# MrTornado24/FENeRF

Hardware: NVIDIA H100
Metric: rendered faces/sec at 128px x 24 samples/ray (higher is better)
Workload: dtype f16 operands / f32 accumulate (wgmma) + f32 refinement

## Files before the change

### fenerf_b200/csrc/siren_fast.cu

```cuda
#include "siren_fast.cuh"

namespace fn {

int siren_fast_label_launch(const void* args, int blocks, cudaStream_t st);
int siren_fast_hd_launch(const void* args, int blocks, bool label_film, cudaStream_t st);
int siren_fast_grid_launch(const void* args, int blocks, cudaStream_t st);
int siren_fast_bridge_launch(const void* args, int blocks, cudaStream_t st);
int siren_fast_debug_launch(const void* args, int blocks, bool label_film, bool feature_head, int variant, cudaStream_t st);

namespace {

std::atomic<int> g_variant{0};
unsigned long long* g_trace = nullptr;
int g_trace_ctas = 0;

bool build_loads(const FnLayout& L, FastArgs& A, bool sigma_only) {
    A.n_loads = 0;
    auto push = [&](size_t src, uint32_t bytes) {
        if (A.n_loads < MAX_LOADS) A.loads[A.n_loads] = Load{(uint32_t)src, bytes};
        ++A.n_loads;
    };
    push(L.first_img, 2 * CHUNK);
    if (L.grid_trunk) push(L.first_img_lo, 2 * CHUNK);
    for (int l = 0; l < L.n_hidden; ++l) {
        if (l == L.trunk_hidden) {
            push(L.head_img, 4 * HEAD_CHUNK);
            if (sigma_only) return A.n_loads <= MAX_LOADS;
        }
        if (L.bridge && l == L.color0) {
            push(L.color0_ximg, 2 * CHUNK);
            continue;
        }
        push(L.hid_img[l], 2 * CHUNK);
        push(L.hid_img[l] + 2 * CHUNK, 2 * CHUNK);
        if (l == L.label_layer) push(L.label.img, (uint32_t)FN_HEAD_IMG_BYTES(L.label.img_rows));
        if (l == L.color0) push(L.color0_ximg, 2 * CHUNK);
        push(L.hid_img[l] + 4 * CHUNK, 2 * CHUNK);
        push(L.hid_img[l] + 6 * CHUNK, 2 * CHUNK);
    }
    push(L.rgb.img, (uint32_t)FN_HEAD_IMG_BYTES(L.rgb.img_rows));
    return A.n_loads <= MAX_LOADS;
}

}

int siren_fast_debug_variant(int variant, unsigned long long* trace, int trace_ctas) {
    FN_REQUIRE(variant >= 0 && variant <= 3, "unknown point-network variant %d", variant);
    FN_REQUIRE(variant < 2 || (trace && trace_ctas >= 1), "a timeline variant needs its trace buffer");
    g_trace = trace;
    g_trace_ctas = trace_ctas;
    g_variant.store(variant);
    return 0;
}

int siren_points_fast(const FnLayout& L, const unsigned char* packed, const float* points, const float* dirs, const float* film,
                      int batch, long long ppb, int dir_group, int lock_dirs, float* out, int sigma_only, cudaStream_t st,
                      float* sigma_out) {
    static_assert(sizeof(FastArgs) <= 4000, "kernel parameter block too large");
    static_assert(SMEM_TOTAL <= 232448, "one CTA per SM: 227 KB of shared memory");
    static_assert(FN_HEAD_IMG_BYTES(FN_FEAT) == SLOT_BYTES, "a feature-head image is one ring slot");
    const bool trunk_only = L.feature_head && sigma_only;
    const bool feature_head = L.feature_head && !trunk_only, label_film = L.label_film && !trunk_only;
    FN_REQUIRE(L.trunk_hidden >= 1 && L.n_hidden - L.color0 >= 1, "field needs >= 2 trunk and >= 1 colour layers");
    FN_REQUIRE(L.sigma_row < 32, "the fast path packs labels and sigma into one 32-column head (label_dim <= 31)");
    FN_REQUIRE(L.rgb.img < 0xFFFFFFFFull && L.label.img < 0xFFFFFFFFull && L.first_img_lo < 0xFFFFFFFFull,
               "packed weight images beyond 4 GB");
    FN_REQUIRE(((uintptr_t)film & 15) == 0, "the FiLM table must be 16-byte aligned");
    if (L.wo_dir && !sigma_only)
        return fail(FENERF_E_UNSUPPORTED, "FENERF_FIELD_WO_DIR: the wgmma colour branch is not accurate for this field (its "
                    "first colour layer amplifies the fp16 trunk's error to ~2e-2 in rgb); render it with "
                    "FENERF_PRECISION_EXACT or FENERF_PRECISION_SPLIT (the density alone runs in any precision)");
    FastArgs a;
    memset(&a, 0, sizeof(a));
    FN_REQUIRE(build_loads(L, a, sigma_only != 0), "field too deep for the weight stream");
    a.sigma_only = sigma_only ? 1 : 0;
    a.L = L; a.packed = packed; a.points = points; a.dirs = dirs; a.film = film; a.out = out; a.sigma_out = sigma_out;
    a.ppb = ppb; a.tiles_per_batch = (ppb + TILE - 1) / TILE; a.n_tiles = a.tiles_per_batch * batch;
    a.dir_group = dir_group < 1 ? 1 : dir_group; a.lock_dirs = lock_dirs;
    if (a.n_tiles <= 0) return 0;
    FN_REQUIRE(ppb % a.dir_group == 0, "points_per_batch %lld not a multiple of dir_group %d", ppb, a.dir_group);
    const long long n_pairs = (a.n_tiles + 1) / 2;
    static std::atomic<int> attr_set[kMaxDevices];
    const int blocks = (int)(n_pairs < (long long)num_sms() ? n_pairs : (long long)num_sms());
    if (const int variant = g_variant.load()) {
        FN_REQUIRE(!L.grid_trunk && !L.bridge,
                   "the debug point-network variants do not cover fields with the grid in the trunk or a bridge");
        a.trace = g_trace;
        a.trace_ctas = g_trace_ctas;
        return siren_fast_debug_launch(&a, blocks, label_film, feature_head, variant, st);
    }
    if (L.grid_trunk) return siren_fast_grid_launch(&a, blocks, st);
    if (L.bridge) return siren_fast_bridge_launch(&a, blocks, st);
    if (feature_head) return siren_fast_hd_launch(&a, blocks, label_film, st);
    if (label_film) return siren_fast_label_launch(&a, blocks, st);
    FN_CUDA_OK(ensure_dynamic_smem(siren_fast_kernel<false>, attr_set, (int)SMEM_TOTAL));
    siren_fast_kernel<false><<<blocks, NTHREADS, SMEM_TOTAL, st>>>(a);
    FN_LAUNCH_OK("siren_fast_kernel");
    return 0;
}

}
```

### fenerf_b200/csrc/siren_fast.cuh

```cuda
#pragma once
#include "common.cuh"
#include "siren_common.cuh"
#include "sm90.cuh"

namespace fn {

namespace {

using namespace sm90;

constexpr int TILE = 64;
constexpr int NTHREADS = 384;
constexpr int PROD_WARP = 8;
constexpr int RING = 6;
constexpr uint32_t SLOT_BYTES = 32768;
constexpr int XSTRIDE = 72;
constexpr uint32_t SMEM_X = RING * SLOT_BYTES;
constexpr int FRING = 2;
constexpr uint32_t FILM_BYTES = 2 * FN_H * 4;
constexpr uint32_t SMEM_FILM = SMEM_X + 2 * TILE * XSTRIDE * 2;
constexpr uint32_t SMEM_BAR = SMEM_FILM + 2 * FRING * FILM_BYTES;
constexpr uint32_t SMEM_TOTAL = SMEM_BAR + 16 * RING + 16 + 16 * 2 * FRING;
constexpr uint32_t SMEM_XLO = SMEM_TOTAL;
constexpr int XLO_STRIDE = 32;
constexpr uint32_t SMEM_TOTAL_GRID = SMEM_XLO + 2 * TILE * XLO_STRIDE * 2;
constexpr int RING_SPLIT = 4;
constexpr uint32_t ALO_CHUNK = TILE * FN_KCHUNK * 2;
constexpr uint32_t ALO_BYTES = (FN_H / FN_KCHUNK) * ALO_CHUNK;
constexpr uint32_t SPLIT_SMEM_ALO = RING_SPLIT * SLOT_BYTES;
constexpr uint32_t SPLIT_SMEM_X = SPLIT_SMEM_ALO + 2 * ALO_BYTES;
constexpr uint32_t SPLIT_SMEM_FILM = SPLIT_SMEM_X + 2 * TILE * XSTRIDE * 2;
constexpr uint32_t SPLIT_SMEM_BAR = SPLIT_SMEM_FILM + 2 * FRING * FILM_BYTES;
constexpr uint32_t SPLIT_SMEM_XLO = SPLIT_SMEM_BAR + 16 * RING_SPLIT + 16 + 16 * 2 * FRING;
constexpr uint32_t SMEM_TOTAL_SPLIT = SPLIT_SMEM_XLO + 2 * TILE * XLO_STRIDE * 2;
constexpr int MAX_LOADS = 72;
constexpr int MAX_LOADS_SPLIT = 132;
constexpr uint32_t CHUNK = 16384;
constexpr uint32_t HEAD_CHUNK = 32 * 128;
constexpr uint32_t RGB_CHUNK = 8 * 128;
constexpr uint32_t FEAT_CHUNK = FN_FEAT * 128;
#ifndef FENERF_SOFT_SIN_EVERY
#define FENERF_SOFT_SIN_EVERY 0
#endif
constexpr int kSoftSinEvery = FENERF_SOFT_SIN_EVERY;
constexpr int kSoftSinSplit = 4;
constexpr int TRACE_CAP = 1024;
constexpr int TRACE_WARPS = 11;
enum TraceEvent {
    TR_PAIR = 1, TR_TURN_WAIT, TR_TURN_DONE, TR_ACQ_WAIT, TR_ACQ_DONE, TR_COMMIT, TR_MMA_DONE, TR_EPI_DONE,
    TR_FILM_WAIT, TR_FILM_DONE, TR_EMPTY_WAIT, TR_EMPTY_DONE,
};
enum TraceGroup { TG_FIRST = 0, TG_HIDDEN, TG_COLOR0, TG_TRUNK_HEAD, TG_LABEL_LAYER, TG_LABEL_HEAD, TG_OUT_HEAD };

__device__ __forceinline__ float soft_sinf(float a) {
    const float k = fmaf(a, 0.159154943f, 12582912.f);
    const float n = k - 12582912.f;
    float r = fmaf(-n, 6.28318548f, a);
    r = fmaf(-n, -1.74845553e-7f, r);
    const float r2 = r * r;
    float p = -2.041572245e-08f;
    p = fmaf(p, r2, 2.701100129e-06f);
    p = fmaf(p, r2, -1.980991656e-04f);
    p = fmaf(p, r2, 8.332454599e-03f);
    p = fmaf(p, r2, -1.666656137e-01f);
    p = fmaf(p, r2, 9.999996424e-01f);
    return r * p;
}

struct Load {
    uint32_t src;
    uint32_t bytes;
};

template <int kMaxLoads>
struct FastArgsT {
    Load loads[kMaxLoads];
    int n_loads;
    FnLayout L;
    const unsigned char* packed;
    const float* points;
    const float* dirs;
    const float* film;
    float* out;
    float* sigma_out;
    long long ppb, tiles_per_batch, n_tiles;
    int dir_group, lock_dirs;
    int sigma_only;
    unsigned long long* trace;
    int trace_ctas;
};
using FastArgs = FastArgsT<MAX_LOADS>;
using SplitArgs = FastArgsT<MAX_LOADS_SPLIT>;

__device__ __forceinline__ void wg_bar(int wg) { asm volatile("bar.sync %0, 128;" ::"r"(1 + wg) : "memory"); }

template <bool kLabelFilm, bool kFeatureHead = false, int kSoftSin = kSoftSinEvery, bool kTrace = false,
          bool kGridTrunk = false, bool kBridge = false, bool kSplit = false>
__global__ void __launch_bounds__(NTHREADS, 1)
    siren_fast_kernel(const __grid_constant__ FastArgsT<kSplit ? MAX_LOADS_SPLIT : MAX_LOADS> a) {
    constexpr int RING = kSplit ? RING_SPLIT : fn::RING;
    constexpr uint32_t SMEM_X = kSplit ? SPLIT_SMEM_X : fn::SMEM_X;
    constexpr uint32_t SMEM_FILM = kSplit ? SPLIT_SMEM_FILM : fn::SMEM_FILM;
    constexpr uint32_t SMEM_BAR = kSplit ? SPLIT_SMEM_BAR : fn::SMEM_BAR;
    constexpr uint32_t SMEM_XLO = kSplit ? SPLIT_SMEM_XLO : fn::SMEM_XLO;
    extern __shared__ __align__(1024) unsigned char smem[];
    const uint32_t sbase = smem_u32(smem);
    const int warp = threadIdx.x >> 5, lane = threadIdx.x & 31;
    const uint32_t bar_full = sbase + SMEM_BAR, bar_empty = bar_full + 8 * RING, bar_turn = bar_empty + 8 * RING;
    const uint32_t bar_ffull = bar_turn + 16, bar_fempty = bar_ffull + 8 * 2 * FRING;
    unsigned long long* tbuf = nullptr;
    uint32_t tn = 0;
    if constexpr (kTrace)
        if (lane == 0 && (int)blockIdx.x < a.trace_ctas) tbuf = a.trace + ((size_t)blockIdx.x * TRACE_WARPS + warp) * TRACE_CAP;
    auto trace = [&](int kind, int group = 0) {
        if constexpr (kTrace)
            if (tbuf && tn < TRACE_CAP)
                tbuf[tn++] = ((unsigned long long)kind << 56) | ((unsigned long long)group << 48) |
                             ((unsigned long long)clock64() & ((1ull << 48) - 1));
    };
    if (threadIdx.x == 0) {
        for (int i = 0; i < RING; ++i) {
            mbar_init(bar_full + 8 * i, 1);
            mbar_init(bar_empty + 8 * i, 8);
        }
        for (int g = 0; g < 2; ++g) mbar_init(bar_turn + 8 * g, 4);
        for (int e = 0; e < 2 * FRING; ++e) {
            mbar_init(bar_ffull + 8 * e, 32);
            mbar_init(bar_fempty + 8 * e, 4);
        }
        fence_barrier_init();
    }
    __syncthreads();
    const long long n_pairs = (a.n_tiles + 1) / 2;

    if (warp >= PROD_WARP) {
        asm volatile("setmaxnreg.dec.sync.aligned.u32 40;\n" ::: "memory");
        if (warp == PROD_WARP && lane == 0) {
            uint32_t it = 0;
            for (long long pair = blockIdx.x; pair < n_pairs; pair += gridDim.x)
                for (int i = 0; i < a.n_loads; ++i, ++it) {
                    const uint32_t slot = it % RING;
                    trace(TR_EMPTY_WAIT);
                    mbar_wait(bar_empty + 8 * slot, ((it / RING) & 1u) ^ 1u);
                    trace(TR_EMPTY_DONE);
                    mbar_arrive_expect_tx(bar_full + 8 * slot, a.loads[i].bytes);
                    bulk_g2s(sbase + slot * SLOT_BYTES, a.packed + a.loads[i].src, a.loads[i].bytes, bar_full + 8 * slot);
                }
        } else if (warp == PROD_WARP + 1 || warp == PROD_WARP + 2) {
            const int g = warp - PROD_WARP - 1;
            const int n_film = 1 + (a.sigma_only ? a.L.trunk_hidden : a.L.n_hidden);
            uint32_t it = 0;
            for (long long pair = blockIdx.x; pair < n_pairs; pair += gridDim.x) {
                const long long tile = pair * 2 + g;
                const long long b = tile < a.n_tiles ? tile / a.tiles_per_batch : 0;
                const float* film_b = a.film + (size_t)b * a.L.n_film * 2 * FN_H;
                for (int i = 0; i < n_film; ++i, ++it) {
                    const uint32_t e = g * FRING + it % FRING;
                    const float2* row = reinterpret_cast<const float2*>(film_b + (size_t)i * 2 * FN_H);
                    const float2* bias = reinterpret_cast<const float2*>(a.packed + (i == 0 ? a.L.first_b : a.L.hid_b[i - 1]));
                    float4* dst = reinterpret_cast<float4*>(smem + SMEM_FILM + e * FILM_BYTES);
                    trace(TR_EMPTY_WAIT);
                    mbar_wait(bar_fempty + 8 * e, ((it / FRING) & 1u) ^ 1u);
                    trace(TR_EMPTY_DONE);
#pragma unroll 1
                    for (int k = 0; k < FN_H / 64; ++k) {
                        const int cp = lane + 32 * k;
                        const float2 f = __ldg(row + cp), p = __ldg(row + FN_H / 2 + cp), bb = __ldg(bias + cp);
                        if constexpr (kSplit) {
                            const float us = __ldg(reinterpret_cast<const float*>(a.packed + a.L.split_scale) +
                                                   FN_SPLIT_SCALES + i);
                            dst[cp] = make_float4(f.x * us, f.y * us, fmaf(f.x, bb.x, p.x), fmaf(f.y, bb.y, p.y));
                        } else {
                            dst[cp] = make_float4(f.x, f.y, fmaf(f.x, bb.x, p.x), fmaf(f.y, bb.y, p.y));
                        }
                    }
                    mbar_arrive(bar_ffull + 8 * e);
                }
            }
        }
        return;
    }

    asm volatile("setmaxnreg.inc.sync.aligned.u32 232;\n" ::: "memory");
    const int wg = warp >> 2, q = lane & 3;
    const int tid = threadIdx.x & 127;
    const int r0 = (warp & 3) * 16 + (lane >> 2);
    const FnLayout& L = a.L;
    const int C = L.out_dim;
    const float* sigma_w = reinterpret_cast<const float*>(a.packed + L.sigma_w);
    const float* label_w = reinterpret_cast<const float*>(a.packed + L.label_w);
    const int trunk_labels = (kLabelFilm || kFeatureHead) ? 0 : L.trunk_labels;
    const int sigma_row = kFeatureHead ? FN_FEAT_SIGMA_ROW : L.sigma_row;
    const int rgb_rows = kFeatureHead ? FN_FEAT : L.rgb.w_rows;
    const int label_rows = kFeatureHead ? FN_FEAT : L.label.w_rows;
    __half* xs = reinterpret_cast<__half*>(smem + SMEM_X) + wg * TILE * XSTRIDE;
    uint32_t it = 0;
    auto acquire = [&](uint32_t& slot) -> uint32_t {
        slot = it % RING;
        trace(TR_ACQ_WAIT);
        mbar_wait(bar_full + 8 * slot, (it / RING) & 1u);
        trace(TR_ACQ_DONE);
        ++it;
        return sbase + slot * SLOT_BYTES;
    };
    auto release = [&](uint32_t slot) {
        __syncwarp();
        if (lane == 0) mbar_arrive(bar_empty + 8 * slot);
    };
    uint32_t turns = 0;
    uint32_t fit = 0;
    auto film_acquire = [&]() -> const float4* {
        const uint32_t e = wg * FRING + fit % FRING;
        trace(TR_FILM_WAIT);
        mbar_wait(bar_ffull + 8 * e, (fit / FRING) & 1u);
        trace(TR_FILM_DONE);
        return reinterpret_cast<const float4*>(smem + SMEM_FILM + e * FILM_BYTES);
    };
    auto film_release = [&]() {
        const uint32_t e = wg * FRING + fit % FRING;
        ++fit;
        __syncwarp();
        if (lane == 0) mbar_arrive(bar_fempty + 8 * e);
    };
    auto turn_begin = [&]() {
        trace(TR_TURN_WAIT);
        mbar_wait(bar_turn + 8 * wg, (turns & 1u) ^ (wg == 0 ? 1u : 0u));
        trace(TR_TURN_DONE);
    };
    auto turn_end = [&](int group) {
        trace(TR_COMMIT, group);
        ++turns;
        __syncwarp();
        if (lane == 0) mbar_arrive(bar_turn + 8 * (wg ^ 1));
    };
    auto xfrag = [&](int s, uint32_t (&f)[4]) {
        const __half* p = xs + r0 * XSTRIDE + 16 * s + 2 * q;
        f[0] = *reinterpret_cast<const uint32_t*>(p);
        f[1] = *reinterpret_cast<const uint32_t*>(p + 8 * XSTRIDE);
        f[2] = *reinterpret_cast<const uint32_t*>(p + 8);
        f[3] = *reinterpret_cast<const uint32_t*>(p + 8 * XSTRIDE + 8);
    };

    for (long long pair = blockIdx.x; pair < n_pairs; pair += gridDim.x) {
        const long long tile = pair * 2 + wg;
        const bool tile_ok = tile < a.n_tiles;
        const long long b = tile_ok ? tile / a.tiles_per_batch : 0;
        const long long p0 = tile_ok ? (tile % a.tiles_per_batch) * TILE : a.ppb;
        trace(TR_PAIR);

        wg_bar(wg);
        if (tid < TILE) {
            float pos[3] = {0.f, 0.f, 0.f}, dir[3] = {0.f, 0.f, 0.f};
            const long long pp = p0 + tid;
            const bool valid = pp < a.ppb;
            if (valid) {
                const long long ff = b * a.ppb + pp;
#pragma unroll
                for (int i = 0; i < 3; ++i) pos[i] = __fmul_rn(a.points[ff * 3 + i], L.input_scale);
                if (a.lock_dirs) dir[2] = -1.f;
                else {
                    const long long di = b * (a.ppb / a.dir_group) + pp / a.dir_group;
#pragma unroll
                    for (int i = 0; i < 3; ++i) dir[i] = a.dirs[di * 3 + i];
                }
            }
            __align__(16) __half slots[64];
#pragma unroll
            for (int i = 0; i < 64; ++i) slots[i] = __float2half_rn(0.f);
#pragma unroll
            for (int i = 0; i < 3; ++i) {
                __half hi, lo;
                split_f16(pos[i], hi, lo);
                slots[FN_SLOT_POS + i] = hi; slots[FN_SLOT_POS + 3 + i] = lo; slots[FN_SLOT_POS + 6 + i] = hi;
                split_f16(dir[i], hi, lo);
                slots[FN_SLOT_DIR + i] = hi; slots[FN_SLOT_DIR + 3 + i] = lo; slots[FN_SLOT_DIR + 6 + i] = hi;
            }
            if constexpr (kGridTrunk || kSplit) {
                __align__(16) __half lo[32];
#pragma unroll
                for (int i = 0; i < 32; ++i) lo[i] = __float2half_rn(0.f);
                if (valid && (kGridTrunk || (L.grid_channels > 0 && !a.sigma_only))) {
                    float feat[32];
                    grid_features32(reinterpret_cast<const float*>(a.packed + L.grid), L.grid_res, pos[0], pos[1], pos[2], feat);
#pragma unroll
                    for (int i = 0; i < 32; ++i) split_f16(feat[i], slots[FN_SLOT_FEAT + i], lo[i]);
                }
                __half* xlo = reinterpret_cast<__half*>(smem + SMEM_XLO) + (wg * TILE + tid) * XLO_STRIDE;
#pragma unroll
                for (int i = 0; i < 4; ++i) reinterpret_cast<uint4*>(xlo)[i] = reinterpret_cast<const uint4*>(lo)[i];
            } else if (L.grid_channels > 0 && valid && !a.sigma_only) {
                float feat[32];
                grid_features32_h(reinterpret_cast<const __half*>(a.packed + L.grid16), L.grid_res, pos[0], pos[1], pos[2], feat);
#pragma unroll
                for (int i = 0; i < 32; ++i) slots[FN_SLOT_FEAT + i] = __float2half_rn(feat[i]);
            }
#pragma unroll
            for (int i = 0; i < 8; ++i)
                reinterpret_cast<uint4*>(xs + tid * XSTRIDE)[i] = reinterpret_cast<const uint4*>(slots)[i];
        }
        wg_bar(wg);

        uint32_t act[16][4];
        uint32_t nxt[8][4];
        float d[64];
        auto film_epi = [&](const float4* fs, int h, uint32_t (&dst)[8][4]) {
#pragma unroll
            for (int j = 0; j < 16; ++j) {
                const float4 e = fs[64 * h + 4 * j + q];
                const bool soft = kSoftSin > 0 && j % (kSoftSin > 0 ? kSoftSin : 1) == kSoftSin - 1;
                auto sn = [soft](float x) { return soft ? soft_sinf(x) : __sinf(x); };
                dst[j >> 1][(j & 1) * 2] = pack_half2(sn(fmaf(e.x, d[4 * j], e.z)), sn(fmaf(e.y, d[4 * j + 1], e.w)));
                dst[j >> 1][(j & 1) * 2 + 1] = pack_half2(sn(fmaf(e.x, d[4 * j + 2], e.z)), sn(fmaf(e.y, d[4 * j + 3], e.w)));
            }
            trace(TR_EPI_DONE);
        };
        auto act_hi = [&]() -> uint32_t (&)[8][4] { return *reinterpret_cast<uint32_t (*)[8][4]>(&act[8]); };
        auto film_epi_split = [&](const float4* fs, int h, uint32_t (&dst)[8][4], uint32_t (&lo)[8][4]) {
#pragma unroll
            for (int j = 0; j < 16; ++j) {
                const float4 e = fs[64 * h + 4 * j + q];
#pragma unroll
                for (int rr = 0; rr < 2; ++rr) {
                    const float s0 = soft_sinf(fmaf(e.x, d[4 * j + 2 * rr], e.z));
                    const float s1 = soft_sinf(fmaf(e.y, d[4 * j + 2 * rr + 1], e.w));
                    const __half2 hi = __floats2half2_rn(s0, s1);
                    const float2 hf = __half22float2(hi);
                    dst[j >> 1][(j & 1) * 2 + rr] = *reinterpret_cast<const uint32_t*>(&hi);
                    lo[j >> 1][(j & 1) * 2 + rr] = pack_half2(s0 - hf.x, s1 - hf.y);
                }
            }
            trace(TR_EPI_DONE);
        };
        const uint32_t alo_base = sbase + SPLIT_SMEM_ALO + wg * ALO_BYTES;
        auto alo_desc = [&](int s) { return desc_kmajor(alo_base + (s >> 2) * ALO_CHUNK + 32 * (s & 3)); };
        auto alo_store = [&](const uint32_t (&lo0)[8][4], const uint32_t (&lo1)[8][4]) {
            wg_bar(wg);
            unsigned char* base = smem + SPLIT_SMEM_ALO + wg * ALO_BYTES;
#pragma unroll
            for (int h = 0; h < 2; ++h)
#pragma unroll
                for (int j = 0; j < 16; ++j) {
                    const int col = 128 * h + 8 * j + 2 * q;
#pragma unroll
                    for (int rr = 0; rr < 2; ++rr)
                        *reinterpret_cast<uint32_t*>(base + (col >> 6) * ALO_CHUNK + fn_sw128_offset(r0 + 8 * rr, col & 63)) =
                            (h ? lo1 : lo0)[j >> 1][(j & 1) * 2 + rr];
                }
            fence_async_smem();
            wg_bar(wg);
        };
        uint32_t lo0[8][4], lo1[8][4];

        {
            uint32_t xf[4], slot, slot_lo = 0, w_lo = 0;
            uint32_t xg[2][4], xl[2][4];
            const float4* fs = nullptr;
            xfrag(0, xf);
            if constexpr (kGridTrunk) {
                const __half* xlo = reinterpret_cast<const __half*>(smem + SMEM_XLO) + wg * TILE * XLO_STRIDE;
#pragma unroll
                for (int s = 0; s < 2; ++s) {
                    xfrag(2 + s, xg[s]);
                    const __half* p = xlo + r0 * XLO_STRIDE + 16 * s + 2 * q;
                    xl[s][0] = *reinterpret_cast<const uint32_t*>(p);
                    xl[s][1] = *reinterpret_cast<const uint32_t*>(p + 8 * XLO_STRIDE);
                    xl[s][2] = *reinterpret_cast<const uint32_t*>(p + 8);
                    xl[s][3] = *reinterpret_cast<const uint32_t*>(p + 8 * XLO_STRIDE + 8);
                }
            }
            const uint32_t w = acquire(slot);
            if constexpr (kGridTrunk) w_lo = acquire(slot_lo);
#pragma unroll
            for (int h = 0; h < 2; ++h) {
                turn_begin();
                wg_fence();
                mma_rs_n128(d, xf, desc_kmajor(w + h * CHUNK), 0u);
                if constexpr (kGridTrunk)
#pragma unroll
                    for (int s = 0; s < 2; ++s) {
                        mma_rs_n128(d, xg[s], desc_kmajor(w + h * CHUNK + 32 * (2 + s)), 1u);
                        mma_rs_n128(d, xl[s], desc_kmajor(w + h * CHUNK + 32 * (2 + s)), 1u);
                        mma_rs_n128(d, xg[s], desc_kmajor(w_lo + h * CHUNK + 32 * (2 + s)), 1u);
                    }
                wg_commit();
                turn_end(TG_FIRST);
                wg_wait<0>();
                trace(TR_MMA_DONE);
                fence_regs(d);
                fence_regs(xf);
                if constexpr (kGridTrunk) { fence_regs(xg); fence_regs(xl); }
                if (h == 0) fs = film_acquire();
                if constexpr (kSplit) {
                    if (h == 0) film_epi_split(fs, 0, nxt, lo0);
                    else film_epi_split(fs, 1, act_hi(), lo1);
                } else {
                    if (h == 0) film_epi(fs, 0, nxt);
                    else film_epi(fs, 1, act_hi());
                }
            }
            release(slot);
            if constexpr (kGridTrunk) release(slot_lo);
            film_release();
            if constexpr (kSplit) alo_store(lo0, lo1);
#pragma unroll
            for (int s = 0; s < 8; ++s)
#pragma unroll
                for (int i = 0; i < 4; ++i) act[s][i] = nxt[s][i];
        }

        bool stop = false;
        for (int l = 0; l < L.n_hidden && !stop; ++l) {
            if (l == L.trunk_hidden) {
                float dh[16];
                uint32_t slot, slot_lo = 0, w_lo = 0;
                const uint32_t w = acquire(slot);
                if constexpr (kSplit) w_lo = acquire(slot_lo);
                turn_begin();
                wg_fence();
#pragma unroll
                for (int c = 0; c < 4; ++c)
#pragma unroll
                    for (int k = 0; k < 4; ++k) mma_rs_n32(dh, act[4 * c + k], desc_kmajor(w + c * HEAD_CHUNK + 32 * k), (c | k) ? 1u : 0u);
                if constexpr (kSplit)
#pragma unroll
                    for (int c = 0; c < 4; ++c)
#pragma unroll
                        for (int k = 0; k < 4; ++k) {
                            mma_ss_n32(dh, alo_desc(4 * c + k), desc_kmajor(w + c * HEAD_CHUNK + 32 * k), 1u);
                            mma_rs_n32(dh, act[4 * c + k], desc_kmajor(w_lo + c * HEAD_CHUNK + 32 * k), 1u);
                        }
                wg_commit();
                turn_end(TG_TRUNK_HEAD);
                wg_wait<0>();
                trace(TR_MMA_DONE);
                fence_regs(dh);
                fence_regs(act);
                release(slot);
                if constexpr (kSplit) {
                    release(slot_lo);
                    const float us = __ldg(reinterpret_cast<const float*>(a.packed + L.split_scale) + FN_SPLIT_SCALES +
                                           L.n_hidden + 1);
#pragma unroll
                    for (int i = 0; i < 16; ++i) dh[i] *= us;
                }
                const float* lb = label_w + FENERF_MAX_LABEL * FN_H;
#pragma unroll
                for (int rr = 0; rr < 2; ++rr) {
                    const long long pnt = p0 + r0 + 8 * rr;
                    if (pnt >= a.ppb) continue;
                    const long long flat = b * a.ppb + pnt;
#pragma unroll
                    for (int i = 0; i < 4; ++i)
#pragma unroll
                        for (int e = 0; e < 2; ++e) {
                            const int o = 8 * i + 2 * q + e;
                            const float v = dh[4 * i + 2 * rr + e];
                            if (o < trunk_labels) {
                                if (!a.sigma_only) a.out[flat * C + o] = fmaf(v, __ldg(lb + FENERF_MAX_LABEL), __ldg(lb + o));
                            } else if (o == sigma_row && !(kBridge && L.bridge_res)) {
                                const float sig = v + __ldg(sigma_w + FN_H);
                                a.out[flat * C + (C - 1)] = sig;
                                if (a.sigma_out) a.sigma_out[flat] = sig;
                            }
                        }
                }
                if constexpr (kBridge) {
                    const float* bw = reinterpret_cast<const float*>(a.packed + L.bridge_w);
#pragma unroll
                    for (int rr = 0; rr < 2; ++rr) {
                        const float o0 = dh[2 * rr], o1 = dh[2 * rr + 1];
                        const float p2 = __shfl_xor_sync(0xffffffffu, o0, 1), p3 = __shfl_xor_sync(0xffffffffu, o1, 1);
                        if (q != 0) continue;
                        const long long pnt = p0 + r0 + 8 * rr;
                        float v[3] = {o1 + __ldg(bw + 3 * FN_H), p2 + __ldg(bw + 3 * FN_H + 1), p3 + __ldg(bw + 3 * FN_H + 2)};
                        if (L.bridge_res) {
                            if (pnt < a.ppb) {
                                const long long flat = b * a.ppb + pnt;
#pragma unroll
                                for (int j = 0; j < 3; ++j) v[j] += __fmul_rn(a.points[flat * 3 + j], L.input_scale);
                                float sig = __ldg(bw + 3 * FN_H + 6);
#pragma unroll
                                for (int j = 0; j < 3; ++j) sig = fmaf(__ldg(bw + 3 * FN_H + 3 + j), v[j], sig);
                                a.out[flat * C + (C - 1)] = sig;
                                if (a.sigma_out) a.sigma_out[flat] = sig;
                            }
                        }
                        if (!a.sigma_only) {
                            __half* row = xs + (r0 + 8 * rr) * XSTRIDE + FN_SLOT_FEAT;
#pragma unroll
                            for (int j = 0; j < 3; ++j) {
                                __half hi, lo;
                                split_f16(v[j], hi, lo);
                                row[j] = hi; row[3 + j] = lo; row[6 + j] = hi;
                            }
                        }
                    }
                    if (!a.sigma_only) wg_bar(wg);
                }
                if (a.sigma_only) { stop = true; break; }
                if constexpr (kLabelFilm) {
                    constexpr int kLabN = kFeatureHead ? FN_FEAT : 32;
                    constexpr uint32_t kLabChunk = kFeatureHead ? FEAT_CHUNK : HEAD_CHUNK;
                    float dl[kLabN / 2];
                    uint32_t slot_h = 0, w_h = 0;
                    const float4* fs = nullptr;
#pragma unroll
                    for (int h = 0; h < 2; ++h) {
                        uint32_t sl[2];
                        turn_begin();
                        wg_fence();
#pragma unroll
                        for (int sb = 0; sb < 2; ++sb) {
                            const uint32_t w = acquire(sl[sb]);
#pragma unroll
                            for (int c = 0; c < 2; ++c)
#pragma unroll
                                for (int k = 0; k < 4; ++k)
                                    mma_rs_n128(d, act[8 * sb + 4 * c + k], desc_kmajor(w + c * CHUNK + 32 * k), (sb | c | k) ? 1u : 0u);
                        }
                        wg_commit();
                        turn_end(TG_LABEL_LAYER);
                        wg_wait<0>();
                        trace(TR_MMA_DONE);
                        fence_regs(d);
                        fence_regs(act);
                        release(sl[0]);
                        release(sl[1]);
                        if (h == 0) fs = film_acquire();
                        film_epi(fs, h, nxt);
                        if (h == 0) w_h = acquire(slot_h);
                        turn_begin();
                        wg_fence();
#pragma unroll
                        for (int s = 0; s < 8; ++s) {
                            const int g = 8 * h + s;
                            const uint64_t desc = desc_kmajor(w_h + (g >> 2) * kLabChunk + 32 * (g & 3));
                            if constexpr (kFeatureHead) mma_rs_n64(dl, nxt[s], desc, (h | s) ? 1u : 0u);
                            else mma_rs_n32(dl, nxt[s], desc, (h | s) ? 1u : 0u);
                        }
                        wg_commit();
                        turn_end(TG_LABEL_HEAD);
                        wg_wait<0>();
                        trace(TR_MMA_DONE);
                        fence_regs(dl);
                        fence_regs(nxt);
                    }
                    release(slot_h);
                    film_release();
#pragma unroll
                    for (int rr = 0; rr < 2; ++rr) {
                        const long long pnt = p0 + r0 + 8 * rr;
                        if (pnt >= a.ppb) continue;
                        const long long flat = b * a.ppb + pnt;
                        const float* lbias = reinterpret_cast<const float*>(a.packed + L.label.w) + label_rows * FN_H;
#pragma unroll
                        for (int i = 0; i < kLabN / 8; ++i)
#pragma unroll
                            for (int e = 0; e < 2; ++e) {
                                const int o = 8 * i + 2 * q + e;
                                if (o < L.label.n_out) a.out[flat * C + o] = dl[4 * i + 2 * rr + e] + __ldg(lbias + o);
                            }
                    }
                    continue;
                }
            }
            const bool c0 = (l == L.color0);
            if constexpr (kSplit) {
                const bool grid = L.grid_channels > 0;
                const float4* fs = nullptr;
#pragma unroll
                for (int h = 0; h < 2; ++h) {
                    uint32_t sl[4], w[4];
#pragma unroll
                    for (int i = 0; i < 4; ++i) w[i] = acquire(sl[i]);
                    turn_begin();
                    wg_fence();
#pragma unroll
                    for (int s = 0; s < 16; ++s)
                        mma_rs_n128(d, act[s], desc_kmajor(w[s >> 3] + ((s >> 2) & 1) * CHUNK + 32 * (s & 3)), s ? 1u : 0u);
#pragma unroll
                    for (int s = 0; s < 16; ++s)
                        mma_ss_n128(d, alo_desc(s), desc_kmajor(w[s >> 3] + ((s >> 2) & 1) * CHUNK + 32 * (s & 3)), 1u);
#pragma unroll
                    for (int s = 0; s < 16; ++s)
                        mma_rs_n128(d, act[s], desc_kmajor(w[2 + (s >> 3)] + ((s >> 2) & 1) * CHUNK + 32 * (s & 3)), 1u);
                    wg_commit();
                    turn_end(c0 ? TG_COLOR0 : TG_HIDDEN);
                    wg_wait<0>();
                    trace(TR_MMA_DONE);
                    fence_regs(d);
                    fence_regs(act);
#pragma unroll
                    for (int i = 0; i < 4; ++i) release(sl[i]);
                    if (c0) {
                        uint32_t xf[3][4], xl[2][4], slot_x, slot_xl = 0, w_xl = 0;
#pragma unroll
                        for (int s = 0; s < 3; ++s) xfrag(1 + s, xf[s]);
                        const __half* xlo = reinterpret_cast<const __half*>(smem + SMEM_XLO) + wg * TILE * XLO_STRIDE;
#pragma unroll
                        for (int s = 0; s < 2; ++s) {
                            const __half* p = xlo + r0 * XLO_STRIDE + 16 * s + 2 * q;
                            xl[s][0] = *reinterpret_cast<const uint32_t*>(p);
                            xl[s][1] = *reinterpret_cast<const uint32_t*>(p + 8 * XLO_STRIDE);
                            xl[s][2] = *reinterpret_cast<const uint32_t*>(p + 8);
                            xl[s][3] = *reinterpret_cast<const uint32_t*>(p + 8 * XLO_STRIDE + 8);
                        }
                        const uint32_t w_x = acquire(slot_x);
                        if (grid) w_xl = acquire(slot_xl);
                        turn_begin();
                        wg_fence();
                        mma_rs_n128(d, xf[0], desc_kmajor(w_x + h * CHUNK + 32), 1u);
                        if (grid)
#pragma unroll
                            for (int s = 0; s < 2; ++s) {
                                const uint32_t off = h * CHUNK + 32 * (2 + s);
                                mma_rs_n128(d, xf[1 + s], desc_kmajor(w_x + off), 1u);
                                mma_rs_n128(d, xl[s], desc_kmajor(w_x + off), 1u);
                                mma_rs_n128(d, xf[1 + s], desc_kmajor(w_xl + off), 1u);
                            }
                        wg_commit();
                        turn_end(TG_COLOR0);
                        wg_wait<0>();
                        trace(TR_MMA_DONE);
                        fence_regs(d);
                        fence_regs(xf);
                        fence_regs(xl);
                        release(slot_x);
                        if (grid) release(slot_xl);
                    }
                    if (h == 0) fs = film_acquire();
                    if (h == 0) film_epi_split(fs, 0, nxt, lo0);
                    else film_epi_split(fs, 1, act_hi(), lo1);
                }
                film_release();
                alo_store(lo0, lo1);
#pragma unroll
                for (int s = 0; s < 8; ++s)
#pragma unroll
                    for (int i = 0; i < 4; ++i) act[s][i] = nxt[s][i];
                continue;
            }
            const bool narrow = kBridge && c0;
            const int nx = kBridge ? 2 : !kGridTrunk && L.grid_channels > 0 ? 3 : 1;
            uint32_t xf[3][4];
            if (c0)
#pragma unroll
                for (int s = 0; s < 3; ++s) xfrag(1 + s, xf[s]);
            uint32_t slot_x = 0, w_x = 0;
            const float4* fs = nullptr;
#pragma unroll
            for (int h = 0; h < 2; ++h) {
                uint32_t sl[2] = {0u, 0u};
                if (narrow && h == 0) w_x = acquire(slot_x);
                turn_begin();
                wg_fence();
                if (!narrow)
#pragma unroll
                    for (int sb = 0; sb < 2; ++sb) {
                        const uint32_t w = acquire(sl[sb]);
#pragma unroll
                        for (int c = 0; c < 2; ++c)
#pragma unroll
                            for (int k = 0; k < 4; ++k)
                                mma_rs_n128(d, act[8 * sb + 4 * c + k], desc_kmajor(w + c * CHUNK + 32 * k), (sb | c | k) ? 1u : 0u);
                    }
                if (c0) {
                    if (h == 0 && !narrow) w_x = acquire(slot_x);
#pragma unroll
                    for (int s = 0; s < 3; ++s)
                        if (s < nx) mma_rs_n128(d, xf[s], desc_kmajor(w_x + h * CHUNK + 32 * (1 + s)), (narrow && s == 0) ? 0u : 1u);
                }
                wg_commit();
                turn_end(c0 ? TG_COLOR0 : TG_HIDDEN);
                wg_wait<0>();
                trace(TR_MMA_DONE);
                fence_regs(d);
                fence_regs(act);
                fence_regs(xf);
                if (!narrow) {
                    release(sl[0]);
                    release(sl[1]);
                }
                if (c0 && h == 1) release(slot_x);
                if (h == 0) fs = film_acquire();
                if (h == 0) film_epi(fs, 0, nxt);
                else film_epi(fs, 1, act_hi());
            }
            film_release();
#pragma unroll
            for (int s = 0; s < 8; ++s)
#pragma unroll
                for (int i = 0; i < 4; ++i) act[s][i] = nxt[s][i];
        }
        if (stop) continue;

        if constexpr (kFeatureHead) {
            float dr[32];
            uint32_t slot;
            const uint32_t w = acquire(slot);
            turn_begin();
            wg_fence();
#pragma unroll
            for (int c = 0; c < 4; ++c)
#pragma unroll
                for (int k = 0; k < 4; ++k) mma_rs_n64(dr, act[4 * c + k], desc_kmajor(w + c * FEAT_CHUNK + 32 * k), (c | k) ? 1u : 0u);
            wg_commit();
            turn_end(TG_OUT_HEAD);
            wg_wait<0>();
            trace(TR_MMA_DONE);
            fence_regs(dr);
            fence_regs(act);
            release(slot);
            const float* rgb_b = reinterpret_cast<const float*>(a.packed + L.rgb.w) + rgb_rows * FN_H;
#pragma unroll
            for (int rr = 0; rr < 2; ++rr) {
                const long long pnt = p0 + r0 + 8 * rr;
                if (pnt >= a.ppb) continue;
                const long long flat = b * a.ppb + pnt;
#pragma unroll
                for (int i = 0; i < 8; ++i)
#pragma unroll
                    for (int e = 0; e < 2; ++e) {
                        const int o = 8 * i + 2 * q + e;
                        a.out[flat * C + L.label_dim + o] = dr[4 * i + 2 * rr + e] + __ldg(rgb_b + o);
                    }
            }
            continue;
        }
        {
            float dr[4];
            uint32_t slot, slot_lo = 0, w_lo = 0;
            const uint32_t w = acquire(slot);
            if constexpr (kSplit) w_lo = acquire(slot_lo);
            turn_begin();
            wg_fence();
#pragma unroll
            for (int c = 0; c < 4; ++c)
#pragma unroll
                for (int k = 0; k < 4; ++k) mma_rs_n8(dr, act[4 * c + k], desc_kmajor(w + c * RGB_CHUNK + 32 * k), (c | k) ? 1u : 0u);
            if constexpr (kSplit)
#pragma unroll
                for (int c = 0; c < 4; ++c)
#pragma unroll
                    for (int k = 0; k < 4; ++k) {
                        mma_ss_n8(dr, alo_desc(4 * c + k), desc_kmajor(w + c * RGB_CHUNK + 32 * k), 1u);
                        mma_rs_n8(dr, act[4 * c + k], desc_kmajor(w_lo + c * RGB_CHUNK + 32 * k), 1u);
                    }
            wg_commit();
            turn_end(TG_OUT_HEAD);
            wg_wait<0>();
            trace(TR_MMA_DONE);
            fence_regs(dr);
            fence_regs(act);
            release(slot);
            if constexpr (kSplit) {
                release(slot_lo);
                const float us = __ldg(reinterpret_cast<const float*>(a.packed + L.split_scale) + FN_SPLIT_SCALES +
                                       L.n_hidden + 2);
#pragma unroll
                for (int i = 0; i < 4; ++i) dr[i] *= us;
            }
            const float* rgb_b = reinterpret_cast<const float*>(a.packed + L.rgb.w) + rgb_rows * FN_H;
#pragma unroll
            for (int rr = 0; rr < 2; ++rr) {
                const long long pnt = p0 + r0 + 8 * rr;
                if (pnt >= a.ppb) continue;
                const long long flat = b * a.ppb + pnt;
#pragma unroll
                for (int e = 0; e < 2; ++e) {
                    const int o = 2 * q + e;
                    if (o < 3) {
                        const float x = dr[2 * rr + e] + __ldg(rgb_b + o);
                        a.out[flat * C + L.label_dim + o] = __fdividef(1.f, 1.f + __expf(-x));
                    }
                }
            }
        }
    }
}

}

}
```

Baseline: 594.8.

## Prefetch tile inputs via bulk copies and release weight slots earlier

Result: no change. 596.4 (median of 6 runs) (+0.3%).

```diff
diff --git a/fenerf_b200/csrc/siren_fast.cu b/fenerf_b200/csrc/siren_fast.cu
--- a/fenerf_b200/csrc/siren_fast.cu
+++ b/fenerf_b200/csrc/siren_fast.cu
@@ -77,6 +77,10 @@
     a.L = L; a.packed = packed; a.points = points; a.dirs = dirs; a.film = film; a.out = out; a.sigma_out = sigma_out;
     a.ppb = ppb; a.tiles_per_batch = (ppb + TILE - 1) / TILE; a.n_tiles = a.tiles_per_batch * batch;
     a.dir_group = dir_group < 1 ? 1 : dir_group; a.lock_dirs = lock_dirs;
+    if (3 * ppb * batch < (1ll << 31)) {
+        a.xin_points = (int)(ppb * batch);
+        a.xin_dirs = a.xin_points / a.dir_group;
+    }
     if (a.n_tiles <= 0) return 0;
     FN_REQUIRE(ppb % a.dir_group == 0, "points_per_batch %lld not a multiple of dir_group %d", ppb, a.dir_group);
     const long long n_pairs = (a.n_tiles + 1) / 2;
diff --git a/fenerf_b200/csrc/siren_fast.cuh b/fenerf_b200/csrc/siren_fast.cuh
--- a/fenerf_b200/csrc/siren_fast.cuh
+++ b/fenerf_b200/csrc/siren_fast.cuh
@@ -20,8 +20,14 @@
 constexpr uint32_t FILM_BYTES = 2 * FN_H * 4;
 constexpr uint32_t SMEM_FILM = SMEM_X + 2 * TILE * XSTRIDE * 2;
 constexpr uint32_t SMEM_BAR = SMEM_FILM + 2 * FRING * FILM_BYTES;
-constexpr uint32_t SMEM_TOTAL = SMEM_BAR + 16 * RING + 16 + 16 * 2 * FRING;
-constexpr uint32_t SMEM_XLO = SMEM_TOTAL;
+constexpr uint32_t SMEM_COMMON = SMEM_BAR + 16 * RING + 16 + 16 * 2 * FRING;
+constexpr int XRING = 2;
+constexpr uint32_t XIN_SPAN = TILE * 12 + 16;
+constexpr uint32_t XIN_BYTES = 2 * XIN_SPAN;
+constexpr uint32_t SMEM_XIN = SMEM_COMMON;
+constexpr uint32_t SMEM_XIN_BAR = SMEM_XIN + 2 * XRING * XIN_BYTES;
+constexpr uint32_t SMEM_TOTAL = SMEM_XIN_BAR + 16 * 2 * XRING;
+constexpr uint32_t SMEM_XLO = SMEM_COMMON;
 constexpr int XLO_STRIDE = 32;
 constexpr uint32_t SMEM_TOTAL_GRID = SMEM_XLO + 2 * TILE * XLO_STRIDE * 2;
 constexpr int RING_SPLIT = 4;
@@ -48,7 +54,7 @@
 constexpr int TRACE_WARPS = 11;
 enum TraceEvent {
     TR_PAIR = 1, TR_TURN_WAIT, TR_TURN_DONE, TR_ACQ_WAIT, TR_ACQ_DONE, TR_COMMIT, TR_MMA_DONE, TR_EPI_DONE,
-    TR_FILM_WAIT, TR_FILM_DONE, TR_EMPTY_WAIT, TR_EMPTY_DONE,
+    TR_FILM_WAIT, TR_FILM_DONE, TR_EMPTY_WAIT, TR_EMPTY_DONE, TR_XIN_WAIT, TR_XIN_DONE,
 };
 enum TraceGroup { TG_FIRST = 0, TG_HIDDEN, TG_COLOR0, TG_TRUNK_HEAD, TG_LABEL_LAYER, TG_LABEL_HEAD, TG_OUT_HEAD };
 
@@ -84,6 +90,7 @@
     float* out;
     float* sigma_out;
     long long ppb, tiles_per_batch, n_tiles;
+    int xin_points, xin_dirs;
     int dir_group, lock_dirs;
     int sigma_only;
     unsigned long long* trace;
@@ -91,6 +98,29 @@
 };
 using FastArgs = FastArgsT<MAX_LOADS>;
 using SplitArgs = FastArgsT<MAX_LOADS_SPLIT>;
+
+struct XinPlan {
+    uint32_t pos_start, dir_start;
+    uint32_t pos_bytes, dir_bytes;
+};
+template <class Args>
+__device__ __forceinline__ bool xin_plan(const Args& a, long long tile, XinPlan& p) {
+    if (a.xin_points == 0 || tile >= a.n_tiles) return false;
+    const uint32_t t = (uint32_t)tile, tpb = (uint32_t)a.tiles_per_batch, ppb = (uint32_t)a.ppb;
+    const uint32_t b = t / tpb, p0 = (t - b * tpb) * TILE;
+    const uint32_t n = ppb - p0 < TILE ? ppb - p0 : TILE, first = b * ppb + p0;
+    auto span = [](const float* base, uint32_t n_all, uint32_t i0, uint32_t i1, uint32_t& start, uint32_t& bytes) {
+        start = (i0 * 3) & ~3u;
+        const uint32_t end = ((i1 + 1) * 3 + 3) & ~3u;
+        bytes = 4 * (end - start);
+        return ((uintptr_t)base & 15) == 0 && end <= n_all * 3;
+    };
+    if (!span(a.points, a.xin_points, first, first + n - 1, p.pos_start, p.pos_bytes)) return false;
+    p.dir_start = 0;
+    p.dir_bytes = 0;
+    const uint32_t g = (uint32_t)a.dir_group;
+    return a.lock_dirs || span(a.dirs, a.xin_dirs, first / g, (first + n - 1) / g, p.dir_start, p.dir_bytes);
+}
 
 __device__ __forceinline__ void wg_bar(int wg) { asm volatile("bar.sync %0, 128;" ::"r"(1 + wg) : "memory"); }
 
@@ -103,11 +133,13 @@
     constexpr uint32_t SMEM_FILM = kSplit ? SPLIT_SMEM_FILM : fn::SMEM_FILM;
     constexpr uint32_t SMEM_BAR = kSplit ? SPLIT_SMEM_BAR : fn::SMEM_BAR;
     constexpr uint32_t SMEM_XLO = kSplit ? SPLIT_SMEM_XLO : fn::SMEM_XLO;
+    constexpr bool kPrefetch = !kGridTrunk && !kSplit;
     extern __shared__ __align__(1024) unsigned char smem[];
     const uint32_t sbase = smem_u32(smem);
     const int warp = threadIdx.x >> 5, lane = threadIdx.x & 31;
     const uint32_t bar_full = sbase + SMEM_BAR, bar_empty = bar_full + 8 * RING, bar_turn = bar_empty + 8 * RING;
     const uint32_t bar_ffull = bar_turn + 16, bar_fempty = bar_ffull + 8 * 2 * FRING;
+    const uint32_t bar_xfull = sbase + SMEM_XIN_BAR, bar_xempty = bar_xfull + 8 * 2 * XRING;
     unsigned long long* tbuf = nullptr;
     uint32_t tn = 0;
     if constexpr (kTrace)
@@ -128,6 +160,11 @@
             mbar_init(bar_ffull + 8 * e, 32);
             mbar_init(bar_fempty + 8 * e, 4);
         }
+        if constexpr (kPrefetch)
+            for (int e = 0; e < 2 * XRING; ++e) {
+                mbar_init(bar_xfull + 8 * e, 1);
+                mbar_init(bar_xempty + 8 * e, 1);
+            }
         fence_barrier_init();
     }
     __syncthreads();
@@ -177,6 +214,22 @@
                     mbar_arrive(bar_ffull + 8 * e);
                 }
             }
+        } else if (kPrefetch && warp == PROD_WARP + 3 && lane == 0) {
+            uint32_t k = 0;
+            for (long long pair = blockIdx.x; pair < n_pairs; pair += gridDim.x, ++k)
+                for (int g = 0; g < 2; ++g) {
+                    const uint32_t e = g * XRING + k % XRING;
+                    mbar_wait(bar_xempty + 8 * e, ((k / XRING) & 1u) ^ 1u);
+                    XinPlan p;
+                    if (xin_plan(a, pair * 2 + g, p)) {
+                        const uint32_t dst = sbase + SMEM_XIN + e * XIN_BYTES;
+                        mbar_arrive_expect_tx(bar_xfull + 8 * e, p.pos_bytes + p.dir_bytes);
+                        bulk_g2s(dst, a.points + p.pos_start, p.pos_bytes, bar_xfull + 8 * e);
+                        if (p.dir_bytes) bulk_g2s(dst + XIN_SPAN, a.dirs + p.dir_start, p.dir_bytes, bar_xfull + 8 * e);
+                    } else {
+                        mbar_arrive(bar_xfull + 8 * e);
+                    }
+                }
         }
         return;
     }
@@ -246,6 +299,8 @@
         const bool tile_ok = tile < a.n_tiles;
         const long long b = tile_ok ? tile / a.tiles_per_batch : 0;
         const long long p0 = tile_ok ? (tile % a.tiles_per_batch) * TILE : a.ppb;
+        const uint32_t xk = (uint32_t)((pair - blockIdx.x) / gridDim.x);
+        const uint32_t xe = wg * XRING + xk % XRING;
         trace(TR_PAIR);
 
         wg_bar(wg);
@@ -253,16 +308,25 @@
             float pos[3] = {0.f, 0.f, 0.f}, dir[3] = {0.f, 0.f, 0.f};
             const long long pp = p0 + tid;
             const bool valid = pp < a.ppb;
+            XinPlan xp{};
+            bool staged = false;
+            if constexpr (kPrefetch) {
+                trace(TR_XIN_WAIT);
+                mbar_wait(bar_xfull + 8 * xe, (xk / XRING) & 1u);
+                trace(TR_XIN_DONE);
+                staged = xin_plan(a, tile, xp);
+            }
+            auto load3 = [&](const float* buf, long long i, uint32_t region, long long start, float (&v)[3]) {
+                const float* s = reinterpret_cast<const float*>(smem + SMEM_XIN + xe * XIN_BYTES + region);
+#pragma unroll
+                for (int c = 0; c < 3; ++c) v[c] = staged ? s[i * 3 - start + c] : buf[i * 3 + c];
+            };
             if (valid) {
-                const long long ff = b * a.ppb + pp;
-#pragma unroll
-                for (int i = 0; i < 3; ++i) pos[i] = __fmul_rn(a.points[ff * 3 + i], L.input_scale);
+                load3(a.points, b * a.ppb + pp, 0, xp.pos_start, pos);
+#pragma unroll
+                for (int i = 0; i < 3; ++i) pos[i] = __fmul_rn(pos[i], L.input_scale);
                 if (a.lock_dirs) dir[2] = -1.f;
-                else {
-                    const long long di = b * (a.ppb / a.dir_group) + pp / a.dir_group;
-#pragma unroll
-                    for (int i = 0; i < 3; ++i) dir[i] = a.dirs[di * 3 + i];
-                }
+                else load3(a.dirs, b * (a.ppb / a.dir_group) + pp / a.dir_group, XIN_SPAN, xp.dir_start, dir);
             }
             __align__(16) __half slots[64];
 #pragma unroll
@@ -299,6 +363,7 @@
                 reinterpret_cast<uint4*>(xs + tid * XSTRIDE)[i] = reinterpret_cast<const uint4*>(slots)[i];
         }
         wg_bar(wg);
+        if (kPrefetch && tid == 0) mbar_arrive(bar_xempty + 8 * xe);
 
         uint32_t act[16][4];
         uint32_t nxt[8][4];
@@ -663,6 +728,7 @@
 #pragma unroll
                             for (int k = 0; k < 4; ++k)
                                 mma_rs_n128(d, act[8 * sb + 4 * c + k], desc_kmajor(w + c * CHUNK + 32 * k), (sb | c | k) ? 1u : 0u);
+                        if (sb == 0) wg_commit();
                     }
                 if (c0) {
                     if (h == 0 && !narrow) w_x = acquire(slot_x);
@@ -672,15 +738,16 @@
                 }
                 wg_commit();
                 turn_end(c0 ? TG_COLOR0 : TG_HIDDEN);
+                if (!narrow) {
+                    wg_wait<1>();
+                    release(sl[0]);
+                }
                 wg_wait<0>();
                 trace(TR_MMA_DONE);
                 fence_regs(d);
                 fence_regs(act);
                 fence_regs(xf);
-                if (!narrow) {
-                    release(sl[0]);
-                    release(sl[1]);
-                }
+                if (!narrow) release(sl[1]);
                 if (c0 && h == 1) release(slot_x);
                 if (h == 0) fs = film_acquire();
                 if (h == 0) film_epi(fs, 0, nxt);
```
